# shunkenney/DPE-MVS

Measured on AMD Instinct MI355X. Metric: depth-map Mpixels/sec (9-view 1600x1200 PatchMatch) at 1/2/4/8 GPUs; L1 vs ref, higher is better.
Workload: dtype f32; 1 GPU; DTU-like 1600x1200, 9 src views, full-res REFINE_ITER pass + geometric consistency (BASELINE configs[2]); width=1600, height=1200, num_images=10, parallelism=reference-image sharding x1

## Files before the change

### dpe-mvs_amd/csrc/dpe_context.h

```cpp
#pragma once
#include <hip/hip_runtime.h>
#include <atomic>
#include <cstdint>
#include <map>
#include <memory>
#include <mutex>
#include <utility>
#include <vector>

#include "pass_common.h"
#include "tap_launch.h"
#include "dpe_fusion_types.h"
#include "cloud_dist.h"

namespace dpe {

inline std::atomic<long long> g_live_bytes{0};

template <class T>
struct DevArr {
  T* p = nullptr;
  size_t n = 0;
  DevArr() = default;
  DevArr(DevArr&& o) noexcept : p(o.p), n(o.n) { o.p = nullptr; o.n = 0; }
// ... 16 lines not shown
  void reset() {
    if (p) { g_live_bytes -= (long long)bytes(); (void)hipFree(p); }
    p = nullptr; n = 0;
  }
};

struct Stream {
  hipStream_t s = nullptr;
  Stream() = default;
  Stream(Stream&& o) noexcept : s(o.s) { o.s = nullptr; }
  Stream(const Stream&) = delete;
  Stream& operator=(const Stream&) = delete;
  ~Stream() { if (s) (void)hipStreamDestroy(s); }
  hipError_t create() { return hipStreamCreateWithFlags(&s, hipStreamNonBlocking); }
  operator hipStream_t() const { return s; }
};
struct Event {
  hipEvent_t e = nullptr;
  Event() = default;
  Event(Event&& o) noexcept : e(o.e) { o.e = nullptr; }
  Event(const Event&) = delete;
  Event& operator=(const Event&) = delete;
  ~Event() { if (e) (void)hipEventDestroy(e); }
  hipError_t create(unsigned flags = hipEventDisableTiming) { return hipEventCreateWithFlags(&e, flags); }
  operator hipEvent_t() const { return e; }
};

struct CachedImage {
  int id = 0, W = 0, H = 0;
  int cls = IMG_F32;
  DevArr<float> plain;
  DevArr<uint32_t> q8;
  DevArr<uint2> q16;
  DevArr<uint32_t> qp;
  DevArr<float4> qf;
  uint64_t last_use = 0;
  size_t bytes() const { return plain.n * 4 + q8.n * 4 + q16.n * 8 + qp.n * 4 + qf.n * 16; }
};

struct ResState {
  int w = 0, h = 0;
  bool full = false;
  DevArr<float4> planes;
  DevArr<uint8_t> weak;
  DevArr<uint32_t> sel;
  DevArr<float> snap;
  int snap_w = 0, snap_h = 0;
  bool has_snap = false;
};

struct PassWork {
  bool staged = false;
#if DPE_GN_ONCE
  bool gn_done_for_stage = false;
  DevArr<float> gn_complex;
#endif
  bool timing = false;
  bool counting = false;
  int gn_slots = 0;
  float timings[DPE_NUM_CLASSES + 1] = {0};
  int launches[DPE_NUM_CLASSES + 1] = {0};
  unsigned long long counts[DPE_NUM_CLASSES * 4] = {0};
  DevArr<unsigned long long> cnt;
  DevArr<unsigned long long> phase;
  PassConst hc;
  DevArr<PassConst> dc;
  DevArr<float> img_plain[DPE_MAX_IMAGES];
  DevArr<float4> imgq[DPE_MAX_IMAGES];
  DevArr<uint32_t> imgq8_all;
  DevArr<uint2> imgq16_all;
  DevArr<uint32_t> imgqp_all;
  int img_cls = IMG_F32;
  DevArr<float> depth[DPE_MAX_IMAGES];
  DevArr<uint8_t> edge, edge_low;
  DevArr<int> label;
  DevArr<float4> planes0;
  DevArr<uint8_t> weak0;
  DevArr<uint32_t> sel0;
  DevArr<float4> planes, planes_snap, fit_plane;
  DevArr<float> costs, costs_snap, complex_;
  DevArr<uint32_t> sel, sel_snap;
  DevArr<uint8_t> weak, weak_rel, vw;
  DevArr<short2> nb, nearest, edge_neigh, lab_bound;
  DevArr<int> radius;
  DevArr<int> tab_right, tab_down;
  DevArr<int> gn_ovf;
  DevArr<float> gn_tab;
  DevArr<int> lists, row_counts, list_totals;
  DevArr<int> part_cnt;
  DevBufs bufs;
};

struct EdgeScratch {
  DevArr<uint8_t> a, b, map;
  DevArr<float> fa, fb;
  DevArr<int> rows, mag, itab;
  DevArr<int16_t> dx, dy;
  DevArr<float> ftab;
  DevArr<short> stab;
};

struct FusionStage {
  std::vector<DevArr<float>> depth, normal;
  std::vector<FusionViewDev> host;
  DevArr<FusionViewDev> views;
  DevArr<DpeCamera> cams;
  DevArr<int> src;
  DevArr<int32_t> idx;
  DevArr<float> val;
  DevArr<uint8_t> cons_count;
  DevArr<float> cons_depth;
  int n = 0;
};

struct TatFusion {
  Event ev;
  std::vector<DevArr<uint8_t>> bgr, block, mask;
  DevArr<TatViewDev> views;
  bool ready = false;
  DevArr<float> dthr;
  DevArr<int> last, agg;
  DevArr<int> cnt, tot;
  DevArr<uint8_t> emit;
  DevArr<TatPoint> rec;
  DevArr<TatPoint> out[2];
  int turn = 0;
  bool copying = false;
  void views_restaged() { ready = false; }
};

struct VizScratch {
  std::mutex mu;
  std::map<const void*, Event> ev;
  DevArr<uint8_t> bgr;
  DevArr<int16_t> blocks;
  DevArr<uint16_t> q;
  int quality = 0;
  DevArr<float4> planes;
  DevArr<uint8_t> weak;
};

struct PointsScratch {
  std::mutex mu;
  std::map<const void*, Event> ev;
  DevArr<uint8_t> bgr;
  DevArr<int> cnt, tot;
  DevArr<TatPoint> out;
  DevArr<float4> planes;
  DevArr<uint8_t> weak;
};

struct CloudTimer {
  std::vector<Event> ev;
  std::vector<int> slot;
  bool on = false;
  float ms[4] = {0, 0, 0, 0};
  bool timed = false;
};
struct VoxelScratch {
  DevArr<uint8_t> rgb;
  DevArr<int4> cell;
  DevArr<uint32_t> frac;
  DevArr<int> owner, count;
  DevArr<uint32_t> first;
  DevArr<unsigned long long> sum, csum;
  DevArr<int> slot_at, bcnt;
// ... 78 lines not shown
```

### dpe-mvs_amd/csrc/dpe_mvs.hip

```cpp
#include <hip/hip_runtime.h>
#include <algorithm>
#include <cmath>
#include <cstdio>
#include <cstring>
#include <string>
#include <memory>
#include <utility>
#include <vector>

#include "pass_tables.h"
#include "pass_kernels.h"
#include "pass_refine.h"
#include "pass_sweep.h"
#include "tap_launch.h"
#include "dpe_entry.h"
#include "dpe_context.h"

using namespace dpe;

static const int kDefaultXcdRows = 1;
static constexpr int kWeakLanes = 16;

thread_local std::string dpe::g_err;

// ... 393 lines not shown
    } else {
      HIPC(c->pass.imgq[i].ensure(plane));
      TRY(build_f32_quads(c->stream, c->pass.img_plain[i].p, W, H, c->pass.imgq[i].p));
      B.imgq[i] = c->pass.imgq[i].p;
    }
  }
  B.ref = c->pass.img_plain[0].p;
  return DPE_OK;
}

static int stage_source_depths(DpeContext* c, const DpePassInput* in, const StageSrc& src) {
  const int W = in->width, H = in->height;
  const size_t L = (size_t)W * H;
  const dim3 rb2(32, 8), rg2((W + 31) / 32, (H + 7) / 8);
  for (int i = 1; i < in->num_images; ++i) {
    HIPC(c->pass.depth[i].ensure(L));
    if (src.st) {
      HIPC(hipMemcpyAsync(c->pass.depth[i].p, in->depths[i], L * sizeof(float), hipMemcpyHostToDevice, c->stream));
    } else {
      const ResState* r = src.dep[i];
      if (src.dep_snap)
        k_rescale_nearest<float><<<rg2, rb2, 0, c->stream>>>(r->snap.p, r->snap_w, r->snap_h, c->pass.depth[i].p, W, H, 0.0f);
      else
        k_rescale_depth<<<rg2, rb2, 0, c->stream>>>(r->planes.p, r->w, r->h, c->pass.depth[i].p, W, H);
      HIPC(hipGetLastError());
    }
    c->pass.bufs.depth[i] = c->pass.depth[i].p;
  }
  return DPE_OK;
}

static int stage_edge_label_maps(DpeContext* c, const DpePassInput* in) {
  const size_t L = (size_t)in->width * in->height, LL = (size_t)in->low_width * in->low_height;
  DevBufs& B = c->pass.bufs;
  if (in->params.use_edge || in->params.use_limit) {
    HIPC(c->pass.edge.ensure(L));
    HIPC(c->pass.edge_low.ensure(LL));
    HIPC(hipMemcpyAsync(c->pass.edge.p, in->edge, L, hipMemcpyHostToDevice, c->stream));
    HIPC(hipMemcpyAsync(c->pass.edge_low.p, in->edge_low_res, LL, hipMemcpyHostToDevice, c->stream));
    B.edge = c->pass.edge.p; B.edge_low = c->pass.edge_low.p;
  }
  if (in->params.use_label) {
    HIPC(c->pass.label.ensure(L));
    HIPC(hipMemcpyAsync(c->pass.label.p, in->label, L * sizeof(int), hipMemcpyHostToDevice, c->stream));
    B.label = c->pass.label.p;
  }
  return DPE_OK;
}

static int stage_initial_state(DpeContext* c, const DpePassInput* in, const StageSrc& src) {
  const DpePatchMatchParams& P = in->params;
  const int W = in->width, H = in->height;
  const size_t L = (size_t)W * H;
  HIPC(c->pass.planes0.ensure(L)); HIPC(c->pass.weak0.ensure(L)); HIPC(c->pass.sel0.ensure(L));
  if (const DpePassState* st = src.st) {
    HIPC(hipMemcpyAsync(c->pass.planes0.p, st->planes, L * sizeof(float4), hipMemcpyHostToDevice, c->stream));
    if (P.use_APD) HIPC(hipMemcpyAsync(c->pass.weak0.p, st->weak_info, L, hipMemcpyHostToDevice, c->stream));
    else HIPC(hipMemsetAsync(c->pass.weak0.p, DPE_STRONG, L, c->stream));
    HIPC(hipMemcpyAsync(c->pass.sel0.p, st->selected_views, L * sizeof(uint32_t), hipMemcpyHostToDevice, c->stream));
    return DPE_OK;
  }
  const ResState* r = src.prior;
  const dim3 rb2(32, 8), rg2((W + 31) / 32, (H + 7) / 8);
  if (P.state != DPE_FIRST_INIT) {
    k_rescale_nearest<float4><<<rg2, rb2, 0, c->stream>>>(r->planes.p, r->w, r->h, c->pass.planes0.p, W, H, make_float4(0, 0, 0, 0));
    k_rescale_nearest<uint32_t><<<rg2, rb2, 0, c->stream>>>(r->sel.p, r->w, r->h, c->pass.sel0.p, W, H, 0u);
  } else {
    HIPC(hipMemsetAsync(c->pass.planes0.p, 0, L * sizeof(float4), c->stream));
    HIPC(hipMemsetAsync(c->pass.sel0.p, 0, L * sizeof(uint32_t), c->stream));
  }
  if (P.use_APD) k_rescale_nearest<uint8_t><<<rg2, rb2, 0, c->stream>>>(r->weak.p, r->w, r->h, c->pass.weak0.p, W, H, (uint8_t)0);
  else HIPC(hipMemsetAsync(c->pass.weak0.p, DPE_STRONG, L, c->stream));
  HIPC(hipGetLastError());
  return DPE_OK;
}

static int ensure_working_set(DpeContext* c, int W, int H) {
  const size_t L = (size_t)W * H;
  HIPC(c->pass.planes.ensure(L)); HIPC(c->pass.planes_snap.ensure(L)); HIPC(c->pass.fit_plane.ensure(L));
  HIPC(c->pass.costs.ensure(L)); HIPC(c->pass.costs_snap.ensure(L)); HIPC(c->pass.complex_.ensure(L));
  HIPC(c->pass.sel.ensure(L)); HIPC(c->pass.sel_snap.ensure(L));
  HIPC(c->pass.weak.ensure(L)); HIPC(c->pass.weak_rel.ensure(L)); HIPC(c->pass.vw.ensure(L * DPE_MAX_IMAGES));
  HIPC(c->pass.nb.ensure(L * 9)); HIPC(c->pass.nearest.ensure(L)); HIPC(c->pass.edge_neigh.ensure(L * 8)); HIPC(c->pass.lab_bound.ensure(L * 8));
  HIPC(c->pass.radius.ensure(L));
  HIPC(c->pass.tab_right.ensure(L)); HIPC(c->pass.tab_down.ensure(L));
  HIPC(c->pass.gn_ovf.ensure(L + 64)); HIPC(c->pass.gn_tab.ensure((size_t)W + H));
  const PassLists lay(W, H, c->pass.hc.half_rows);
  HIPC(c->pass.lists.ensure((size_t)lay.lists_len())); HIPC(c->pass.row_counts.ensure(lay.row_counts_len()));
  HIPC(c->pass.list_totals.ensure(PassLists::kTotals)); HIPC(c->pass.part_cnt.ensure(lay.part_cnt_len()));
  DevBufs& B = c->pass.bufs;
  B.planes = c->pass.planes.p; B.planes_snap = c->pass.planes_snap.p; B.fit_plane = c->pass.fit_plane.p;
  B.planes0 = c->pass.planes0.p;
  B.costs = c->pass.costs.p; B.costs_snap = c->pass.costs_snap.p; B.complex_ = c->pass.complex_.p;
  B.sel = c->pass.sel.p; B.sel_snap = c->pass.sel_snap.p;
  B.weak = c->pass.weak.p; B.weak_rel = c->pass.weak_rel.p; B.vw = c->pass.vw.p;
  B.nb = c->pass.nb.p; B.nearest = c->pass.nearest.p; B.edge_neigh = c->pass.edge_neigh.p; B.lab_bound = c->pass.lab_bound.p;
  B.radius = c->pass.radius.p;
  return DPE_OK;
}

static int stage_impl(DpeContext* c, const DpePassInput* in, const StageSrc& src) {
  Range range_(src.st ? "dpe_pm_stage" : "dpe_pm_stage_resident");
  TRY(stage_check_args(in));
  HIPC(hipSetDevice(c->device));
  HIPC(wait_pending(c));
  set_pass_constants(c->pass.hc, in);
  HIPC(c->pass.dc.ensure(1));
  HIPC(hipMemcpyAsync(c->pass.dc.p, &c->pass.hc, sizeof(PassConst), hipMemcpyHostToDevice, c->stream));
  std::memset(&c->pass.bufs, 0, sizeof(c->pass.bufs));
  TRY(in->image_ids ? stage_images_cached(c, in) : stage_images_direct(c, in));
  if (in->params.geom_consistency) TRY(stage_source_depths(c, in, src));
  TRY(stage_edge_label_maps(c, in));
  TRY(stage_initial_state(c, in, src));
  TRY(ensure_working_set(c, in->width, in->height));
  HIPC(hipStreamSynchronize(c->stream));
  c->pass.staged = true;
#if DPE_GN_ONCE
  c->pass.gn_done_for_stage = false;
#endif
  return DPE_OK;
}

extern "C" int dpe_pm_stage(DpeContext* c, const DpePassInput* in, const DpePassState* st) {
  g_err.clear();
  if (!c || !in || !st || !in->images || !in->cams || !st->planes || !st->weak_info || !st->selected_views) {
    g_err = "dpe_pm_stage: null argument"; return DPE_ERR_ARG;
  }
  if (in->params.geom_consistency) {
    if (!in->depths) { g_err = "dpe_pm_stage: geom_consistency needs depths"; return DPE_ERR_ARG; }
    for (int i = 1; i < in->num_images; ++i) if (!in->depths[i]) { g_err = "dpe_pm_stage: missing source depth"; return DPE_ERR_ARG; }
  }
  StageSrc src;
  src.st = st;
  return stage_impl(c, in, src);
}

extern "C" int dpe_pm_stage_resident(DpeContext* c, const DpePassInput* in, int prior_id) {
  g_err.clear();
  if (!c || !in || !in->images || !in->cams) { g_err = "dpe_pm_stage_resident: null argument"; return DPE_ERR_ARG; }
  const DpePatchMatchParams& P = in->params;
  StageSrc src;
  auto find = [&](int id) -> const ResState* { auto it = c->rstore.find(id); return it == c->rstore.end() ? nullptr : &it->second; };
  if (P.state != DPE_FIRST_INIT || P.use_APD) {
    src.prior = find(prior_id);
    if (!src.prior || !src.prior->full) {
      g_err = "dpe_pm_stage_resident: no resident state of image " + std::to_string(prior_id); return DPE_ERR_STATE;
    }
  }
  if (P.geom_consistency) {
    if (!in->image_ids) { g_err = "dpe_pm_stage_resident: geom_consistency needs image_ids"; return DPE_ERR_ARG; }
    for (int i = 1; i < in->num_images && i < DPE_MAX_IMAGES; ++i) {
      src.dep[i] = find(in->image_ids[i]);
      if (!src.dep[i]) { g_err = "no depth map of source image " + std::to_string(in->image_ids[i]); return DPE_ERR_STATE; }
    }
    src.dep_snap = c->snap_mode;
    if (src.dep_snap)
      for (int i = 1; i < in->num_images && i < DPE_MAX_IMAGES; ++i)
        if (!src.dep[i]->has_snap) { g_err = "no depth snapshot of source image " + std::to_string(in->image_ids[i]); return DPE_ERR_STATE; }
  }
  return stage_impl(c, in, src);
}


static const char* const kClassName[DPE_NUM_CLASSES] = {"setup", "init", "strong", "ransac", "weak", "filter",
                                                         "depth_to_weak", "local_refine"};

struct PassRecorder {
  DpeContext* c = nullptr;
  hipStream_t s = nullptr;
  const DevBufs* base = nullptr;
  bool timing = false, slot_overflow = false;
  int max_slots = 0, nev = 0;
  std::vector<int> ev_class;

  int start(DpeContext* c_, hipStream_t s_, DevBufs& B) {
    c = c_; s = s_; base = &B;
    timing = c->pass.timing;
#if DPE_PHASE_PROF
    HIPC(c->pass.phase.ensure(32 * 64));
// ... 52 lines not shown
      }
    }
#if DPE_PHASE_PROF
    unsigned long long ph32[32 * 64], ph[64] = {};
    HIPC(hipMemcpyAsync(ph32, c->pass.phase.p, sizeof(ph32), hipMemcpyDeviceToHost, s));
    HIPC(hipStreamSynchronize(s));
    for (int k = 0; k < 32 * 64; ++k) ph[k % 64] += ph32[k];
    unsigned long long tot[4] = {0, 0, 0, 0};
    for (int k = 0; k < 64; ++k) tot[k / 16] += ph[k];
    for (int k = 0; k < 64; ++k)
      if (ph[k]) fprintf(stderr, "PHASE %d.%d %.4e cycles %.1f%%\n", k / 16, k % 16, (double)ph[k], 100.0 * ph[k] / tot[k / 16]);
#endif
    if (c->pass.counting) {
      HIPC(hipMemcpyAsync(c->pass.counts, c->pass.cnt.p, sizeof(c->pass.counts), hipMemcpyDeviceToHost, s));
      HIPC(hipStreamSynchronize(s));
      for (int k = 0; k < DPE_NUM_CLASSES; ++k) c->pass.counts[4 * k + 3] = (unsigned long long)c->pass.launches[k];
    }
    return DPE_OK;
  }
};
using Section = PassRecorder::Section;

struct PassRun {
  DpeContext* c;
  hipStream_t s, a;
  bool overlap;
  const PassConst& pc;
  const PassConst* dpc;
  DevBufs B;
  PassLists lay;
  size_t L;
  int nv;
  bool gn_skip = false;
  PassRecorder rec;

  PassRun(DpeContext* c_, hipStream_t s_)
      : c(c_), s(s_), a(s_), pc(c_->pass.hc), dpc(c_->pass.dc.p), B(c_->pass.bufs), lay(pc.W, pc.H, pc.half_rows),
        L((size_t)pc.W * pc.H), nv(pc.N - 1) {
    static const bool overlap_env = [] { const char* e = getenv("DPE_OVERLAP"); return !(e && atoi(e) == 0); }();
    overlap = overlap_env && !c->pass.timing && !c->pass.counting && pc.P.max_iterations >= 1;
    if (overlap) a = c->aux;
    B.cnt = nullptr;
    const char* e = getenv("DPE_XCD_ROWS");
    B.xcd_rows = e ? atoi(e) : kDefaultXcdRows;
  }
  hipError_t fork(hipEvent_t ev) const {
    const hipError_t e = overlap ? hipEventRecord(ev, s) : hipSuccess;
    return e != hipSuccess || !overlap ? e : hipStreamWaitEvent(a, ev, 0);
  }
  hipError_t aux_done(hipEvent_t ev) const { return overlap ? hipEventRecord(ev, a) : hipSuccess; }
  hipError_t wait_aux(hipEvent_t ev) const { return overlap ? hipStreamWaitEvent(s, ev, 0) : hipSuccess; }
  hipError_t join(hipEvent_t ev) const { const hipError_t e = aux_done(ev); return e != hipSuccess ? e : wait_aux(ev); }

  int* list(PassLists::Region r) const { return c->pass.lists.p + r.off; }
  int* rows(PassLists::Region r) const { return c->pass.row_counts.p + r.off; }
  int* total(int slot) const { return c->pass.list_totals.p + slot; }
  int* chunk_counts(int colour) const { return c->pass.part_cnt.p + lay.chunk_counts(colour).off; }
  dim3 px_grid() const { return dim3((pc.W + 15) / 16, (pc.H + 15) / 16); }
};
static const dim3 kPxBlock(16, 16);

template <int MODE>
static void build_lists(const PassRun& X, hipStream_t st, const DevBufs& Bl, PassLists::Region rows, int total,
                        PassLists::Region list) {
  const unsigned grid = (unsigned)(((MODE == 1 ? X.pc.H : X.pc.half_rows) + 3) / 4);
  const long stride = MODE == 1 ? X.lay.px() : list.len;
  int* rc = X.rows(rows);
  k_list_count<MODE><<<grid, 256, 0, st>>>(X.dpc, Bl, rc);
  k_list_scan<MODE><<<1, 64 * list_count<MODE>(), 0, st>>>(X.dpc, rc, X.total(total));
  k_list_fill<MODE><<<grid, 256, 0, st>>>(X.dpc, Bl, rc, X.list(list), stride);
}
static void sweep_lists(const PassRun& X, const DevBufs& Bl) {
  build_lists<0>(X, X.s, Bl, X.lay.sweep_rows(), PassLists::total_sweep(0, 0), X.lay.sweep(0, 0));
}

static int clear_setup_state(const PassRun& X, hipStream_t st) {
  const DevBufs& B = X.B;
  const size_t L = X.L;
  HIPC(hipMemsetAsync(B.fit_plane, 0, L * sizeof(float4), st));
  HIPC(hipMemsetAsync(B.complex_, 0, L * sizeof(float), st));
  if (!X.gn_skip) HIPC(hipMemsetAsync(B.weak_rel, 0xFF, L, st));
  if (!X.gn_skip) HIPC(hipMemsetAsync(B.nb, 0xFF, L * 9 * sizeof(short2), st));
  HIPC(hipMemsetAsync(B.nearest, 0xFF, L * sizeof(short2), st));
  HIPC(hipMemsetAsync(B.edge_neigh, 0xFF, L * 8 * sizeof(short2), st));
  HIPC(hipMemsetAsync(B.lab_bound, 0xFF, L * 8 * sizeof(short2), st));
  HIPC(hipMemsetAsync(B.radius, 0, L * sizeof(int), st));
  return DPE_OK;
}

static int gen_neighbours(PassRun& X, const DevBufs& Bc) {
  DpeContext* c = X.c;
  const hipStream_t a = X.a;
  const int* weak_list = X.list(X.lay.all_weak());
  const int* cnt = X.total(PassLists::kTotAllWeak);
  if (X.gn_skip) {
  } else if (X.pc.P.rotate_time <= 4) {
    int* ovf = X.total(PassLists::kTotGnOverflow);
    k_gn_tables<<<(unsigned)((X.pc.W + X.pc.H + 255) / 256), 256, 0, a>>>(X.dpc, c->pass.gn_tab.p);
    HIPC(hipMemsetAsync(ovf, 0, sizeof(int), a));
    const unsigned gg = (unsigned)((X.L + kGnBT - 1) / kGnBT);
    if (c->pass.gn_slots == 8)
      k_gen_neighbours_lds<8><<<gg, kGnBT, 0, a>>>(X.dpc, Bc, weak_list, cnt, c->pass.gn_tab.p, c->pass.gn_ovf.p, ovf);
    else if (X.pc.P.rotate_time <= 2 && c->pass.gn_slots != 64)
      k_gen_neighbours_lds<32><<<gg, kGnBT, 0, a>>>(X.dpc, Bc, weak_list, cnt, c->pass.gn_tab.p, c->pass.gn_ovf.p, ovf);
    else
      k_gen_neighbours_lds<64><<<gg, kGnBT, 0, a>>>(X.dpc, Bc, weak_list, cnt, c->pass.gn_tab.p, c->pass.gn_ovf.p, ovf);
    k_gen_neighbours<<<kGnOvfBlocks, 256, 0, a>>>(X.dpc, Bc, c->pass.gn_ovf.p, ovf);
  } else {
    k_gen_neighbours<<<kGnOvfBlocks, 256, 0, a>>>(X.dpc, Bc, weak_list, cnt);
  }
#if DPE_GN_ONCE
  if (!X.gn_skip) {
    HIPC(c->pass.gn_complex.ensure(X.L));
    HIPC(hipMemcpyAsync(c->pass.gn_complex.p, X.B.complex_, X.L * sizeof(float), hipMemcpyDeviceToDevice, a));
    c->pass.gn_done_for_stage = true;
  }
#endif
  return DPE_OK;
}

static int setup_chain(PassRun& X) {
  DpeContext* c = X.c;
  const PassConst& pc = X.pc;
  const hipStream_t a = X.a;
  Section sec(X.rec, DPE_CLASS_SETUP);
  const DevBufs& Bc = sec.B;
  if (X.overlap) sweep_lists(X, Bc);
  HIPC(X.fork(c->ev_fork));
  TRY(clear_setup_state(X, a));
  k_gen_edge_inform<<<X.px_grid(), kPxBlock, 0, a>>>(X.dpc, Bc);
  if (pc.P.use_edge) k_edge_rays<<<(unsigned)(3 * (pc.W + pc.H) - 2), 64, 0, a>>>(X.dpc, Bc);
#if DPE_GN_ONCE
  if (X.gn_skip) HIPC(hipMemcpyAsync(X.B.complex_, c->pass.gn_complex.p, X.L * sizeof(float), hipMemcpyDeviceToDevice, a));
#endif
  HIPC(X.aux_done(c->ev_ei));
  k_strong_tables_scan<<<(unsigned)(pc.W + pc.H), 64, 0, a>>>(X.dpc, Bc, c->pass.tab_right.p, c->pass.tab_down.p);
  k_find_nearest_strong<<<X.px_grid(), kPxBlock, 0, a>>>(X.dpc, Bc, c->pass.tab_right.p, c->pass.tab_down.p);
  build_lists<1>(X, a, Bc, X.lay.all_weak_rows(), PassLists::kTotAllWeak, X.lay.all_weak());
  TRY(gen_neighbours(X, Bc));
  k_neighbour_update<<<X.px_grid(), kPxBlock, 0, a>>>(X.dpc, Bc);
  if (X.overlap) build_lists<2>(X, a, Bc, X.lay.failed_rows(), PassLists::kTotFailed, X.lay.failed());
  else sweep_lists(X, Bc);
  HIPC(X.aux_done(c->ev_join));
  return DPE_OK;
}

static int random_initialization(PassRun& X) {
  {
    Section sec(X.rec, DPE_CLASS_INIT);
    if (X.c->pass.img_cls != IMG_F32) k_random_init<kTexInit><<<X.px_grid(), kPxBlock, 0, X.s>>>(X.dpc, sec.B);
    else k_random_init<TEX_F32><<<X.px_grid(), kPxBlock, 0, X.s>>>(X.dpc, sec.B);
  }
  HIPC(X.wait_aux(X.c->ev_ei));
  HIPC(hipGetLastError());
  return DPE_OK;
}

static void strong_sweep(const PassRun& X, const DevBufs& Bs, int it, PassLists::Region list, int total) {
  const bool edge = X.pc.P.use_edge;
  const int P = edge ? 4 : 8, C = edge ? 16 : 8;
  const size_t lds = (size_t)kBwStrong * strong_lds_per_wave(P, C, X.nv) * sizeof(float);
  const unsigned grid = (unsigned)((X.L / 2 + 1 + kBwStrong * P - 1) / (kBwStrong * P));
  launch_strong(edge, X.c->pass.img_cls, grid, lds, X.s, X.dpc, Bs, it, X.list(list), X.total(total));
}

static int strong_half_sweep(PassRun& X, int it, int colour) {
  const DevBufs& B = X.B;
// ... 174 lines not shown
```

### dpe-mvs_amd/csrc/pass_common.h

```cpp
#pragma once
#include "device_math.h"
#include "bres_walk.h"
#include "tex_addr.h"
#include "../../include/dpe_mvs.h"

namespace dpe {

struct ViewConst { float M[9]; float b[3]; };

struct PassConst {
  int W, H, N, LW, LH;
  int half_rows;
  uint32_t seed32, salt;
  float kinv0, kinv4, kc2, kc5;
  float gn_cos, gn_sin, gn_thr;
  int gn_shift;
  uint32_t gn_shift_m;
  int weak_nn;
  int tex_wide;
  float base_len[DPE_MAX_IMAGES];
  float spat36[36];
  DpePatchMatchParams P;
  DpeCamera cams[DPE_MAX_IMAGES];
  ViewConst vc[DPE_MAX_IMAGES];
};

struct DevBufs {
  const float4* imgq[DPE_MAX_IMAGES];
  const uint8_t* img8; uint32_t img8_view;
  const uint8_t* img16; uint32_t img16_view;
  const uint8_t* imgp; uint32_t imgp_view;
  const float* depth[DPE_MAX_IMAGES];
  const float* ref;
  float4* planes; float4* planes_snap; float4* fit_plane;
  const float4* planes0;
  float* costs; float* costs_snap; float* complex_;
  uint32_t* sel; uint32_t* sel_snap;
  uint8_t* weak; uint8_t* weak_rel; uint8_t* vw;
  short2* nb; short2* nearest; short2* edge_neigh; short2* lab_bound;
  int* radius;
  const uint8_t* edge; const uint8_t* edge_low; const int* label;
  unsigned long long* cnt;
  unsigned long long* phase;
  int xcd_rows;
};

#ifndef DPE_DIAG
#define DPE_DIAG 0
#endif
#define DPE_POOL_STATS (((DPE_DIAG) >> 4) & 1)
#define DPE_PHASE_PROF ((DPE_DIAG) & 1)
#define DPE_LINE_STATS (((DPE_DIAG) >> 1) & 1)
#define DPE_WEAK_STATS (((DPE_DIAG) >> 2) & 1)
#define DPE_GN_TIMES (((DPE_DIAG) >> 3) & 1)
#define DPE_FAKE_GATHER (((DPE_DIAG) >> 5) & 1)
#define DPE_GN_ONCE (((DPE_DIAG) >> 6) & 1)
#if DPE_PHASE_PROF
#define PHASE_BEGIN() uint64_t ph_t_ = __builtin_readcyclecounter(), ph_acc_[16] = {}
#define PHASE(k)                                                                    \
  do {                                                                              \
    const uint64_t n_ = __builtin_readcyclecounter();                               \
    ph_acc_[k] += n_ - ph_t_;                                                       \
    ph_t_ = n_;                                                                     \
  } while (0)
#define PHASE_END(kernel)                                                           \
  do {                                                                              \
    if ((threadIdx.x & 63) == 0 && B.phase)                                         \
      for (int k_ = 0; k_ < 16; ++k_)                                               \
        if (ph_acc_[k_]) atomicAdd(B.phase + ((blockIdx.x & 31) * 4 + (kernel)) * 16 + k_, (unsigned long long)ph_acc_[k_]); \
  } while (0)
#define PHASE_END_ALL(kernel)                                                       \
  do {                                                                              \
    if (B.phase)                                                                    \
      for (int k_ = 0; k_ < 16; ++k_)                                               \
        if (ph_acc_[k_]) atomicAdd(B.phase + ((blockIdx.x & 31) * 4 + (kernel)) * 16 + k_, (unsigned long long)ph_acc_[k_]); \
  } while (0)
#else
#define PHASE_BEGIN() do {} while (0)
#define PHASE(k) do {} while (0)
#define PHASE_END(kernel) do {} while (0)
#define PHASE_END_ALL(kernel) do {} while (0)
#endif
#if DPE_POOL_STATS
static __device__ unsigned long long g_pool[8][3];
DEV void pool_stat(int k, int jobs) {
  if ((threadIdx.x & 63) == 0) {
    atomicAdd(&g_pool[k][0], (unsigned long long)jobs);
    atomicAdd(&g_pool[k][1], (unsigned long long)((jobs + 63) / 64));
    atomicAdd(&g_pool[k][2], 1ull);
  }
}
#define POOL_STAT(k, n) pool_stat(k, n)
#define PATCH_STAT(ok) do { atomicAdd(&g_pool[6][0], 1ull); if (!(ok)) atomicAdd(&g_pool[6][1], 1ull); } while (0)
#else
#define POOL_STAT(k, n) do {} while (0)
#define PATCH_STAT(ok) do {} while (0)
#endif
DEV void count_work(const DevBufs& B, unsigned long long ncc, unsigned long long taps) {
  if (B.cnt) { atomicAdd(B.cnt + 0, ncc); atomicAdd(B.cnt + 1, taps); }
}

DEV int xcd_remap(int b, int nb, int chunk) {
  if (chunk <= 0) return b;
  const int super = 8 * chunk;
  const int S = (nb / super) * super;
  if (b >= S) return b;
  const int xcd = b & 7, pos = b >> 3;
  return ((pos / chunk) * 8 + xcd) * chunk + (pos % chunk);
}

DEV void setBit(uint32_t& v, unsigned n) { v |= (1u << n); }
DEV void unSetBit(uint32_t& v, unsigned n) { v &= (0xFFFFFFFEu << n); }
DEV int isSet(uint32_t v, unsigned n) { return (v >> n) & 1; }

DEV void normalize3(float4& v) {
  const float n2 = v.x * v.x + v.y * v.y + v.z * v.z;
  const float inv = d_rsqrtf(n2);
  v.x *= inv; v.y *= inv; v.z *= inv;
}
DEV void normalize2(float2& v) {
  const float n2 = v.x * v.x + v.y * v.y;
  const float inv = d_rsqrtf(n2);
// ... 749 lines not shown
```

### dpe-mvs_amd/csrc/pass_kernels.h

```cpp
#pragma once
#include "pass_common.h"

namespace dpe {

#define PIX2D_FULL()                                                   \
  const int lb_ = xcd_remap(blockIdx.y * gridDim.x + blockIdx.x, gridDim.x * gridDim.y, B.xcd_rows * gridDim.x); \
  const int x = (lb_ % gridDim.x) * blockDim.x + threadIdx.x;          \
  const int y = (lb_ / gridDim.x) * blockDim.y + threadIdx.y;          \
  if (x >= pc.W || y >= pc.H) return;                                  \
  const int center = x + y * pc.W;

#define PIX2D_HALF()                                                   \
  const int lb_ = xcd_remap(blockIdx.y * gridDim.x + blockIdx.x, gridDim.x * gridDim.y, B.xcd_rows * gridDim.x); \
  const int y = (lb_ / gridDim.x) * blockDim.y + threadIdx.y;          \
  const int x = 2 * ((lb_ % gridDim.x) * blockDim.x + threadIdx.x) + ((y + colour) & 1); \
  if (x >= pc.W || y >= pc.H || y >= pc.half_rows) return;             \
  const int center = x + y * pc.W;

constexpr int kEiTileR = 8, kEiTile = 16 + 2 * kEiTileR;
__global__ void __launch_bounds__(64) k_edge_rays(const PassConst* __restrict__ pcp, DevBufs B) {
  const PassConst& pc = *pcp;
  const int W = pc.W, H = pc.H;
  const int lane = threadIdx.x;
  int line = blockIdx.x;
  int f, x0, y0, sx, sy, len, iprev, inext;
  if (line < H) { f = 0; x0 = 0; y0 = line; sx = 1; sy = 0; len = W; iprev = 2; inext = 3; }
  else if ((line -= H) < W) { f = 1; x0 = line; y0 = 0; sx = 0; sy = 1; len = H; iprev = 0; inext = 1; }
  else if ((line -= W) < W + H - 1) {
    f = 2; const int c = line - (H - 1);
    y0 = c < 0 ? -c : 0; x0 = c + y0; sx = 1; sy = 1; len = MINo(H - y0, W - x0); iprev = 4; inext = 5;
  } else {
    line -= W + H - 1; f = 3; const int sm = line;
    y0 = sm - (W - 1) > 0 ? sm - (W - 1) : 0; x0 = sm - y0; sx = -1; sy = 1; len = MINo(H - y0, x0 + 1); iprev = 7; inext = 6;
  }
  (void)f;
  const unsigned long long below = lane == 0 ? 0ull : (~0ull >> (64 - lane));
  const unsigned long long above = lane == 63 ? 0ull : (~0ull << (lane + 1));
  int carry = -1;
  for (int t0 = 0; t0 < len; t0 += 64) {
    const int t = t0 + lane;
    const int px = x0 + t * sx, py = y0 + t * sy;
    const bool e = t < len && B.edge[py * W + px] != 0;
    const unsigned long long m = __ballot(e);
    const unsigned long long lo = m & below;
    const int prev = lo ? t0 + 63 - __builtin_clzll(lo) : carry;
    if (t < len) {
      B.edge_neigh[(size_t)(py * W + px) * 8 + iprev] =
          prev < 0 ? make_short2(-1, -1) : make_short2((short)(x0 + prev * sx), (short)(y0 + prev * sy));
    }
    if (m) carry = t0 + 63 - __builtin_clzll(m);
  }
  carry = -1;
  for (int t0 = ((len - 1) / 64) * 64; t0 >= 0; t0 -= 64) {
    const int t = t0 + lane;
    const int px = x0 + t * sx, py = y0 + t * sy;
    const bool e = t < len && B.edge[py * W + px] != 0;
    const unsigned long long m = __ballot(e);
    const unsigned long long hi = m & above;
    const int next = hi ? t0 + __builtin_ctzll(hi) : carry;
    if (t < len) {
      B.edge_neigh[(size_t)(py * W + px) * 8 + inext] =
          next < 0 ? make_short2(-1, -1) : make_short2((short)(x0 + next * sx), (short)(y0 + next * sy));
    }
    if (m) carry = t0 + __builtin_ctzll(m);
  }
}

__global__ void __launch_bounds__(256) k_gen_edge_inform(const PassConst* __restrict__ pcp, DevBufs B) {
  const PassConst& pc = *pcp;
  __shared__ uint8_t s_tile[kEiTile * kEiTile];
  __shared__ uint32_t s_hs[kEiTile][16];
  const int radius = pc.P.strong_radius;
  const bool tiled = pc.P.use_edge && radius >= 0 && radius <= kEiTileR && blockDim.x == 16;
  if (tiled) {
    const int lb0 = xcd_remap(blockIdx.y * gridDim.x + blockIdx.x, gridDim.x * gridDim.y, B.xcd_rows * gridDim.x);
    const int ox = (lb0 % gridDim.x) * blockDim.x - radius, oy = (lb0 / gridDim.x) * blockDim.y - radius;
    const int tw = blockDim.x + 2 * radius, th = blockDim.y + 2 * radius;
    for (int t = threadIdx.y * blockDim.x + threadIdx.x; t < tw * th; t += blockDim.x * blockDim.y) {
      const int nx = ox + t % tw, ny = oy + t / tw;
      uint8_t v = 0;
      if (nx >= 0 && nx < pc.W && ny >= 0 && ny < pc.H) {
        const int q = ny * pc.W + nx;
        v = 4 | (B.edge[q] ? 1 : 0) | ((pc.P.use_label && B.label[q] == 0) ? 2 : 0);
      }
      s_tile[t] = v;
    }
    __syncthreads();
    for (int t = threadIdx.y * blockDim.x + threadIdx.x; t < th * 16; t += blockDim.x * blockDim.y) {
      const uint8_t* row = s_tile + (t / 16) * tw + t % 16;
      uint32_t acc = 0;
      for (int i = 0; i <= 2 * radius; i++) {
        const uint32_t v = row[i];
        acc += (v & 1u) | ((v & 2u) << 9) | ((v & 4u) << 18);
      }
      s_hs[t / 16][t % 16] = acc;
    }
    __syncthreads();
  }
  PIX2D_FULL();
  const int W = pc.W, H = pc.H;
  if (pc.P.use_edge) {
    int edge_pix = 0, tot_pix = 0, bound_pix = 0;
    if (tiled) {
      uint32_t acc = 0;
      for (int j = 0; j <= 2 * radius; j++) acc += s_hs[threadIdx.y + j][threadIdx.x];
      edge_pix = (int)(acc & 1023u); bound_pix = (int)((acc >> 10) & 1023u); tot_pix = (int)(acc >> 20);
    } else {
      for (int i = -radius; i <= radius; i++)
        for (int j = -radius; j <= radius; j++) {
          const int nx = x + i, ny = y + j;
          if (nx < 0 || nx >= W || ny < 0 || ny >= H) continue;
          if (B.edge[ny * W + nx]) edge_pix++;
          if (pc.P.use_label && B.label[ny * W + nx] == 0) bound_pix++;
          tot_pix++;
        }
    }
    float density = 1.0f * edge_pix / tot_pix;
    if (pc.P.use_label) density = MAXo(density, (float)(bound_pix / tot_pix));
    B.complex_[center] = (float)(1.0f / (1.0f + d_exp_d(-25.0 * ((double)density - 0.35))));
  }
  if (pc.P.use_label && B.weak[center] == DPE_WEAK) {
    const int cl = B.label[center];
    if (cl > 0) {
      short2* lb = B.lab_bound + (size_t)center * 8;
      for (int i = 0; i < 8; i++) {
        const int dx = kDir[i][0], dy = kDir[i][1];
        const int sx = dx > 0 ? W - 1 - x : (dx < 0 ? x : 1 << 30);
        const int sy = dy > 0 ? H - 1 - y : (dy < 0 ? y : 1 << 30);
        const int n = MINo(sx, sy);
        int lk = -1;
        bool stop = false;
        for (int k0 = 1; k0 <= n && !stop; k0 += 8) {
          int lab[8];
#pragma unroll
          for (int k = 0; k < 8; ++k) lab[k] = (k0 + k <= n) ? B.label[(x + (k0 + k) * dx) + (y + (k0 + k) * dy) * W] : -1;
#pragma unroll
          for (int k = 0; k < 8; ++k) {
            if (stop) continue;
            if (k0 + k > n) { stop = true; continue; }
            if (lab[k] == cl) lk = k0 + k;
            else if (lab[k] == -1) stop = true;
          }
        }
        lb[i] = lk < 0 ? make_short2(-1, -1) : make_short2((short)(x + lk * dx), (short)(y + lk * dy));
      }
// ... 927 lines not shown
```

### dpe-mvs_amd/csrc/pass_sweep.h

```cpp
#pragma once
#include "pass_common.h"
#include "pass_refine.h"
#include "lds_layout.h"
#include "pass_lists.h"
#include "pool_tail.h"

namespace dpe {

template <int MODE> constexpr int list_count() { return MODE == 0 ? 4 : 1; }
template <int MODE> DEV int list_rows(const PassConst& pc) { return MODE == 1 ? pc.H : pc.half_rows; }
template <int MODE> DEV int list_key(const PassConst& pc, const DevBufs& B, int x, int y) {
  if constexpr (MODE == 2) return (((x + y) & 1) == 0 && B.weak_rel[y * pc.W + x] == 0) ? 0 : -1;
  const bool wk = B.weak[y * pc.W + x] == DPE_WEAK;
  if constexpr (MODE == 1) return wk ? 0 : -1;
  else return (((x + y) & 1) << 1) | (wk ? 1 : 0);
}
template <int MODE>
__global__ void k_list_count(const PassConst* __restrict__ pcp, DevBufs B, int* __restrict__ row_counts) {
  constexpr int NL = list_count<MODE>();
  const PassConst& pc = *pcp;
  const int wave = threadIdx.x >> 6, lane = threadIdx.x & 63;
  const int y = blockIdx.x * 4 + wave, rows = list_rows<MODE>(pc);
  if (y >= rows) return;
  int cnt[NL];
// ... 115 lines not shown
  int runA = 0;
  for (int i0 = base; i0 < min(n, base + kPartChunk); i0 += 256) {
    const int i = i0 + (int)threadIdx.x;
    const int p = i < n ? list[i] : 0;
    const int k = i < n ? part_key(pc, B, p) : 0;
    const unsigned long long m = __ballot(k == 1);
    if (lane == 0) s4[wave] = __popcll(m);
    __syncthreads();
    int a = runA + __popcll(m & below);
    for (int w = 0; w < wave; ++w) a += s4[w];
    const int all = s4[0] + s4[1] + s4[2] + s4[3];
    __syncthreads();
    if (i < n) out[k ? offA + a : offB + (i - base) - a] = p;
    runA += all;
  }
}

template <class CostF>
DEV float view_prob_raw(CostF cost, int i, float cost_threshold) {
  float count = 0; int count_false = 0; float tmpw = 0;
#pragma unroll
  for (int j = 0; j < 8; j++) {
    const float c = cost(j, i);
    if (c < cost_threshold) { tmpw += d_expf(c * c / (-0.18f)); count++; }
    if (c > 1.2f) count_false++;
  }
  float sp = 0.0f;
  if (count > 2 && count_false < 3) sp = tmpw / count;
  else if (count_false < 3) sp = d_expf(cost_threshold * cost_threshold / (-0.32f));
  return sp;
}

DEV void view_sample(const float* sp, int nv, Rng& rs, uint8_t* vw, uint32_t& tsv, float& wnorm) {
  for (int i = 0; i < DPE_MAX_IMAGES; ++i) vw[i] = 0;
  float psum = 0.0f;
  for (int i = 0; i < nv; ++i) psum += sp[i];
  const float inv = 1.0f / psum;
  float cdf[DPE_MAX_IMAGES];
  float cum = 0.0f;
  for (int i = 0; i < nv; ++i) { const float q = sp[i] * inv; cum += q; cdf[i] = cum; }
  for (int s = 0; s < 15; ++s) {
    const float rp = rng_uniform(rs) - 1.1920929e-07f;
    for (int id = 0; id < nv; ++id)
      if (cdf[id] > rp) { vw[id] += 1; break; }
  }
  uint32_t t = 0; float wn = 0;
  for (int i = 0; i < nv; ++i) if (vw[i] > 0) { setBit(t, i); wn += vw[i]; }
  tsv = t; wnorm = wn;
}

DEV void view_sample_coop(float* sp, int* cnt, int nv, int c, int C, bool active, const Rng& rs, uint8_t* vwl,
                          uint8_t* vwg) {
  if (active) {
    if (c == 0) {
      float psum = 0.0f;
      for (int i = 0; i < nv; ++i) psum += sp[i];
      const float inv = 1.0f / psum;
      float cum = 0.0f;
      for (int i = 0; i < nv; ++i) { const float q = sp[i] * inv; cum += q; sp[i] = cum; }
    }
    for (int v = c; v < nv; v += C) cnt[v] = 0;
  }
  wave_sync();
  if (active) {
    for (int s = c; s < 15; s += C) {
      const float rp = u32_to_uniform(rng_word(rs, (uint32_t)s)) - 1.1920929e-07f;
      for (int id = 0; id < nv; ++id)
        if (sp[id] > rp) { atomicAdd(&cnt[id], 1); break; }
    }
  }
  wave_sync();
  if (active)
    for (int j = c; j < DPE_MAX_IMAGES; j += C) {
      const uint8_t w = j < nv ? (uint8_t)cnt[j] : (uint8_t)0;
      vwl[j] = w;
      vwg[j] = w;
    }
  wave_sync();
}

DEV int edge_candidate(const PassConst& pc, const DevBufs& B, const float* __restrict__ costs, int x, int y, int center,
                       int iter, int d, int kind, bool on_edge) {
  const int W = pc.W, H = pc.H;
  const int dx = kDir[d][0], dy = kDir[d][1];
  const int s0 = MAXo(1, 5 - 2 * iter);
  const int min_step_len = 2;
  int step_num = 11, step_len = min_step_len;
  if (kind == 0) {
    const float max_edge_dist = MAXo(H, W) / 30.0f;
    const short2 ep = B.edge_neigh[(size_t)center * 8 + d];
    const double ex = (double)(ep.x - x), ey = (double)(ep.y - y);
    float dist = (float)__builtin_sqrt(ex * ex + ey * ey);
    if (d >= 4) dist = (float)((double)dist / 1.4142135623730951);
    if (on_edge) dist = 11 * min_step_len;
    else if (ep.x == -1 || ep.y == -1 || dist > max_edge_dist) {
      dist = max_edge_dist;
      if (d >= 4) dist = (float)((double)dist / 1.4142135623730951);
    }
    step_num = MINo(MAXo(11, f2i(1.0f * dist / min_step_len)), 22);
    step_len = MAXo(f2i(1.0f * dist / step_num), min_step_len);
    if (d < 4 && step_len % 2 == 1) step_len -= 1;
  }
  int fx = 0, fy = 0;
  if (d > 4) { if (d % 2) fx = dx; else fy = dy; }
  int mpos = -1; float mc = 3.40282347e+38f;
  for (int s = 0; s < step_num; s += 8) {
    float cv[8]; int pv[8]; bool ok[8];
#pragma unroll
    for (int u = 0; u < 8; ++u) {
      const int step = s + u;
      const int tx = x + s0 * dx + step * step_len * dx + fx, ty = y + s0 * dy + step * step_len * dy + fy;
      ok[u] = step < step_num && tx >= 0 && ty >= 0 && tx < W && ty < H;
      pv[u] = tx + ty * W;
      cv[u] = ok[u] ? costs[pv[u]] : 0.0f;
    }
#pragma unroll
    for (int u = 0; u < 8; ++u)
      if (ok[u] && mc > cv[u]) { mpos = pv[u]; mc = cv[u]; }
  }
  return mc < 3.40282347e+38f ? mpos : -1;
}

DEV int acmh_candidate(const PassConst& pc, const float* __restrict__ costs, int x, int y, int center, int s) {
  const int W = pc.W, H = pc.H;
  float costMin; int cmp;
  switch (s) {
    case 1: {
      if (!(y > 2)) return -1;
      const int up_far = center - 3 * W; costMin = costs[up_far]; cmp = up_far;
      for (int i = 1; i < 11; ++i) if (y > 2 + 2 * i) { const int pt = up_far - 2 * i * W; if (costs[pt] < costMin) { costMin = costs[pt]; cmp = pt; } }
      return cmp;
    }
    case 3: {
      if (!(y < H - 3)) return -1;
      const int down_far = center + 3 * W; costMin = costs[down_far]; cmp = down_far;
      for (int i = 1; i < 11; ++i) if (y < H - 3 - 2 * i) { const int pt = down_far + 2 * i * W; if (costs[pt] < costMin) { costMin = costs[pt]; cmp = pt; } }
      return cmp;
    }
    case 5: {
      if (!(x > 2)) return -1;
      const int left_far = center - 3; costMin = costs[left_far]; cmp = left_far;
      for (int i = 1; i < 11; ++i) if (x > 2 + 2 * i) { const int pt = left_far - 2 * i; if (costs[pt] < costMin) { costMin = costs[pt]; cmp = pt; } }
      return cmp;
    }
    case 7: {
      if (!(x < W - 3)) return -1;
      const int right_far = center + 3; costMin = costs[right_far]; cmp = right_far;
      for (int i = 1; i < 11; ++i) if (x < W - 3 - 2 * i) { const int pt = right_far + 2 * i; if (costs[pt] < costMin) { costMin = costs[pt]; cmp = pt; } }
      return cmp;
    }
    case 0: {
      if (!(y > 0)) return -1;
      const int up_near = center - W; costMin = costs[up_near]; cmp = up_near;
      for (int i = 0; i < 3; ++i) {
        if (y > 1 + i && x > i) { const int pt = up_near - (1 + i) * W - (1 + i); if (costs[pt] < costMin) { costMin = costs[pt]; cmp = pt; } }
        if (y > 1 + i && x < W - 1 - i) { const int pt = up_near - (1 + i) * W + (1 + i); if (costs[pt] < costMin) { costMin = costs[pt]; cmp = pt; } }
      }
      return cmp;
    }
    case 2: {
      if (!(y < H - 1)) return -1;
      const int down_near = center + W; costMin = costs[down_near]; cmp = down_near;
      for (int i = 0; i < 3; ++i) {
        if (y < H - 2 - i && x > i) { const int pt = down_near + (1 + i) * W - (1 + i); if (costs[pt] < costMin) { costMin = costs[pt]; cmp = pt; } }
        if (y < H - 2 - i && x < W - 1 - i) { const int pt = down_near + (1 + i) * W + (1 + i); if (costs[pt] < costMin) { costMin = costs[pt]; cmp = pt; } }
      }
      return cmp;
    }
    case 4: {
      if (!(x > 0)) return -1;
      const int left_near = center - 1; costMin = costs[left_near]; cmp = left_near;
      for (int i = 0; i < 3; ++i) {
        if (x > 1 + i && y > i) { const int pt = left_near - (1 + i) - (1 + i) * W; if (costs[pt] < costMin) { costMin = costs[pt]; cmp = pt; } }
        if (x > 1 + i && y < H - 1 - i) { const int pt = left_near - (1 + i) + (1 + i) * W; if (costs[pt] < costMin) { costMin = costs[pt]; cmp = pt; } }
      }
      return cmp;
    }
    default: {
      if (!(x < W - 1)) return -1;
      const int right_near = center + 1; costMin = costs[right_near]; cmp = right_near;
      for (int i = 0; i < 3; ++i) {
        if (x < W - 2 - i && y > i) { const int pt = right_near + (1 + i) - (1 + i) * W; if (costs[pt] < costMin) { costMin = costs[pt]; cmp = pt; } }
        if (x < W - 2 - i && y < H - 1 - i) { const int pt = right_near + (1 + i) + (1 + i) * W; if (costs[pt] < costMin) { costMin = costs[pt]; cmp = pt; } }
      }
      return cmp;
    }
  }
}

constexpr int kTailJobs = kTailLdsJobs;
template <int P, int C> using StrongCarveT = lds::StrongCarve<P, C, kTailJobs>;
__host__ __device__ inline int strong_lds_per_wave(int P, int C, int nv) {
  return P == 4 && C == 16 ? StrongCarveT<4, 16>::total(nv) : StrongCarveT<8, 8>::total(nv);
}
template <int P, int C>
struct StrongWave {
  using SC = StrongCarveT<P, C>;
  float* wl;
  int nv;
  DEV float4* hyp(int q) const { return (float4*)(wl + SC::hyp()) + q * 5; }
  DEV float* patch(int q) const { return wl + SC::patch() + q * SC::kPatch; }
  DEV float* cost(int q) const { return wl + SC::cost(nv) + q * (C + 1) * nv; }
  DEV float* sp(int q) const { return wl + SC::sp(nv) + q * nv; }
// ... 1110 lines not shown
```

Baseline: 31.72 Mpix/s.

## Precompute edge-scan step geometry in scan kernel and use prefix bounds in candidate search

The edge-scan kernel now derives each pixel's step count and step length from the distance to the nearest edge along each direction. It uses a shared-memory lookup table indexed by distance and stores the result as a packed 16-bit value per pixel and direction. edge_candidate reads this packed value instead of loading edge_neigh and computing sqrt and divisions per candidate. It also computes the in-bounds step prefix once, so the per-step bounds checks go away and the last valid load is clamped. The memset of edge_neigh is dropped, and the scan kernel writes an extra buffer.

```diff
diff --git a/dpe-mvs_amd/csrc/dpe_context.h b/dpe-mvs_amd/csrc/dpe_context.h
--- a/dpe-mvs_amd/csrc/dpe_context.h
+++ b/dpe-mvs_amd/csrc/dpe_context.h
@@ -122,6 +122,7 @@
   DevArr<uint32_t> sel, sel_snap;
   DevArr<uint8_t> weak, weak_rel, vw;
   DevArr<short2> nb, nearest, edge_neigh, lab_bound;
+  DevArr<uint16_t> scan_geo;
   DevArr<int> radius;
   DevArr<int> tab_right, tab_down;
   DevArr<int> gn_ovf;
diff --git a/dpe-mvs_amd/csrc/dpe_mvs.hip b/dpe-mvs_amd/csrc/dpe_mvs.hip
--- a/dpe-mvs_amd/csrc/dpe_mvs.hip
+++ b/dpe-mvs_amd/csrc/dpe_mvs.hip
@@ -499,6 +499,7 @@
   HIPC(c->pass.sel.ensure(L)); HIPC(c->pass.sel_snap.ensure(L));
   HIPC(c->pass.weak.ensure(L)); HIPC(c->pass.weak_rel.ensure(L)); HIPC(c->pass.vw.ensure(L * DPE_MAX_IMAGES));
   HIPC(c->pass.nb.ensure(L * 9)); HIPC(c->pass.nearest.ensure(L)); HIPC(c->pass.edge_neigh.ensure(L * 8)); HIPC(c->pass.lab_bound.ensure(L * 8));
+  HIPC(c->pass.scan_geo.ensure(L * 8));
   HIPC(c->pass.radius.ensure(L));
   HIPC(c->pass.tab_right.ensure(L)); HIPC(c->pass.tab_down.ensure(L));
   HIPC(c->pass.gn_ovf.ensure(L + 64)); HIPC(c->pass.gn_tab.ensure((size_t)W + H));
@@ -512,6 +513,7 @@
   B.sel = c->pass.sel.p; B.sel_snap = c->pass.sel_snap.p;
   B.weak = c->pass.weak.p; B.weak_rel = c->pass.weak_rel.p; B.vw = c->pass.vw.p;
   B.nb = c->pass.nb.p; B.nearest = c->pass.nearest.p; B.edge_neigh = c->pass.edge_neigh.p; B.lab_bound = c->pass.lab_bound.p;
+  B.scan_geo = c->pass.scan_geo.p;
   B.radius = c->pass.radius.p;
   return DPE_OK;
 }
@@ -730,7 +732,6 @@
   if (!X.gn_skip) HIPC(hipMemsetAsync(B.weak_rel, 0xFF, L, st));
   if (!X.gn_skip) HIPC(hipMemsetAsync(B.nb, 0xFF, L * 9 * sizeof(short2), st));
   HIPC(hipMemsetAsync(B.nearest, 0xFF, L * sizeof(short2), st));
-  HIPC(hipMemsetAsync(B.edge_neigh, 0xFF, L * 8 * sizeof(short2), st));
   HIPC(hipMemsetAsync(B.lab_bound, 0xFF, L * 8 * sizeof(short2), st));
   HIPC(hipMemsetAsync(B.radius, 0, L * sizeof(int), st));
   return DPE_OK;
diff --git a/dpe-mvs_amd/csrc/pass_common.h b/dpe-mvs_amd/csrc/pass_common.h
--- a/dpe-mvs_amd/csrc/pass_common.h
+++ b/dpe-mvs_amd/csrc/pass_common.h
@@ -2,6 +2,7 @@
 #include "device_math.h"
 #include "bres_walk.h"
 #include "tex_addr.h"
+#include "scan_geo.h"
 #include "../../include/dpe_mvs.h"
 
 namespace dpe {
@@ -38,6 +39,7 @@
   uint32_t* sel; uint32_t* sel_snap;
   uint8_t* weak; uint8_t* weak_rel; uint8_t* vw;
   short2* nb; short2* nearest; short2* edge_neigh; short2* lab_bound;
+  uint16_t* scan_geo;
   int* radius;
   const uint8_t* edge; const uint8_t* edge_low; const int* label;
   unsigned long long* cnt;
diff --git a/dpe-mvs_amd/csrc/pass_kernels.h b/dpe-mvs_amd/csrc/pass_kernels.h
--- a/dpe-mvs_amd/csrc/pass_kernels.h
+++ b/dpe-mvs_amd/csrc/pass_kernels.h
@@ -33,7 +33,16 @@
     line -= W + H - 1; f = 3; const int sm = line;
     y0 = sm - (W - 1) > 0 ? sm - (W - 1) : 0; x0 = sm - y0; sx = -1; sy = 1; len = MINo(H - y0, x0 + 1); iprev = 7; inext = 6;
   }
-  (void)f;
+  __shared__ uint16_t s_geo[kScanLutMax];
+  const int dcls = f >= 2 ? 4 : 0;
+  const int nfar = scan_geo_far_len(W, H), nlut = MINo(nfar, kScanLutMax);
+  for (int n = lane; n < nlut; n += 64) s_geo[n] = scan_geo_pack(edge_scan_geometry(W, H, 0, 0, n, f >= 2 ? n : 0, dcls));
+  const uint16_t geo_far = scan_geo_pack(edge_scan_geometry(W, H, 0, 0, -1, -1, dcls));
+  __syncthreads();
+  auto geo_at = [&](int n) -> uint16_t {
+    if (n < 0 || n >= nfar) return geo_far;
+    return n < nlut ? s_geo[n] : scan_geo_pack(edge_scan_geometry(W, H, 0, 0, n, f >= 2 ? n : 0, dcls));
+  };
   const unsigned long long below = lane == 0 ? 0ull : (~0ull >> (64 - lane));
   const unsigned long long above = lane == 63 ? 0ull : (~0ull << (lane + 1));
   int carry = -1;
@@ -45,8 +54,9 @@
     const unsigned long long lo = m & below;
     const int prev = lo ? t0 + 63 - __builtin_clzll(lo) : carry;
     if (t < len) {
-      B.edge_neigh[(size_t)(py * W + px) * 8 + iprev] =
-          prev < 0 ? make_short2(-1, -1) : make_short2((short)(x0 + prev * sx), (short)(y0 + prev * sy));
+      const short2 ep = prev < 0 ? make_short2(-1, -1) : make_short2((short)(x0 + prev * sx), (short)(y0 + prev * sy));
+      B.edge_neigh[(size_t)(py * W + px) * 8 + iprev] = ep;
+      B.scan_geo[(size_t)(py * W + px) * 8 + iprev] = geo_at(prev < 0 ? -1 : t - prev);
     }
     if (m) carry = t0 + 63 - __builtin_clzll(m);
   }
@@ -59,8 +69,9 @@
     const unsigned long long hi = m & above;
     const int next = hi ? t0 + __builtin_ctzll(hi) : carry;
     if (t < len) {
-      B.edge_neigh[(size_t)(py * W + px) * 8 + inext] =
-          next < 0 ? make_short2(-1, -1) : make_short2((short)(x0 + next * sx), (short)(y0 + next * sy));
+      const short2 ep = next < 0 ? make_short2(-1, -1) : make_short2((short)(x0 + next * sx), (short)(y0 + next * sy));
+      B.edge_neigh[(size_t)(py * W + px) * 8 + inext] = ep;
+      B.scan_geo[(size_t)(py * W + px) * 8 + inext] = geo_at(next < 0 ? -1 : next - t);
     }
     if (m) carry = t0 + __builtin_ctzll(m);
   }
diff --git a/dpe-mvs_amd/csrc/pass_sweep.h b/dpe-mvs_amd/csrc/pass_sweep.h
--- a/dpe-mvs_amd/csrc/pass_sweep.h
+++ b/dpe-mvs_amd/csrc/pass_sweep.h
@@ -221,43 +221,30 @@
 DEV int edge_candidate(const PassConst& pc, const DevBufs& B, const float* __restrict__ costs, int x, int y, int center,
                        int iter, int d, int kind, bool on_edge) {
   const int W = pc.W, H = pc.H;
-  const int dx = kDir[d][0], dy = kDir[d][1];
   const int s0 = MAXo(1, 5 - 2 * iter);
-  const int min_step_len = 2;
-  int step_num = 11, step_len = min_step_len;
-  if (kind == 0) {
-    const float max_edge_dist = MAXo(H, W) / 30.0f;
-    const short2 ep = B.edge_neigh[(size_t)center * 8 + d];
-    const double ex = (double)(ep.x - x), ey = (double)(ep.y - y);
-    float dist = (float)__builtin_sqrt(ex * ex + ey * ey);
-    if (d >= 4) dist = (float)((double)dist / 1.4142135623730951);
-    if (on_edge) dist = 11 * min_step_len;
-    else if (ep.x == -1 || ep.y == -1 || dist > max_edge_dist) {
-      dist = max_edge_dist;
-      if (d >= 4) dist = (float)((double)dist / 1.4142135623730951);
-    }
-    step_num = MINo(MAXo(11, f2i(1.0f * dist / min_step_len)), 22);
-    step_len = MAXo(f2i(1.0f * dist / step_num), min_step_len);
-    if (d < 4 && step_len % 2 == 1) step_len -= 1;
-  }
-  int fx = 0, fy = 0;
-  if (d > 4) { if (d % 2) fx = dx; else fy = dy; }
-  int mpos = -1; float mc = 3.40282347e+38f;
-  for (int s = 0; s < step_num; s += 8) {
-    float cv[8]; int pv[8]; bool ok[8];
+  ScanGeo g{kScanFixedNum, kScanFixedLen};
+  if (kind == 0 && !on_edge) g = scan_geo_unpack(B.scan_geo[(size_t)center * 8 + d]);
+  int dx, dy;
+  scan_dir(d, dx, dy);
+  const int kmax = scan_prefix(x, y, d, s0, g.step_len, g.step_num, W, H);
+  const int dpos = dx + dy * W;
+  int p0 = center + s0 * dpos;
+  if (d > 4) p0 += (d & 1) ? dx : dy * W;
+  const int stride = g.step_len * dpos;
+  const int p0b = p0 * 4, strideb = stride * 4;
+  uint32_t moff = 0; float mc = 3.40282347e+38f;
+  for (int s = 0; s < kmax; s += 8) {
+    float cv[8]; uint32_t off[8];
 #pragma unroll
     for (int u = 0; u < 8; ++u) {
-      const int step = s + u;
-      const int tx = x + s0 * dx + step * step_len * dx + fx, ty = y + s0 * dy + step * step_len * dy + fy;
-      ok[u] = step < step_num && tx >= 0 && ty >= 0 && tx < W && ty < H;
-      pv[u] = tx + ty * W;
-      cv[u] = ok[u] ? costs[pv[u]] : 0.0f;
+      off[u] = (uint32_t)(p0b + __mul24(MINo(s + u, kmax - 1), strideb));
+      cv[u] = *(const float*)((const char*)costs + off[u]);
     }
 #pragma unroll
     for (int u = 0; u < 8; ++u)
-      if (ok[u] && mc > cv[u]) { mpos = pv[u]; mc = cv[u]; }
-  }
-  return mc < 3.40282347e+38f ? mpos : -1;
+      if (mc > cv[u]) { moff = off[u]; mc = cv[u]; }
+  }
+  return mc < 3.40282347e+38f ? (int)(moff >> 2) : -1;
 }
 
 DEV int acmh_candidate(const PassConst& pc, const float* __restrict__ costs, int x, int y, int center, int s) {
diff --git a/dpe-mvs_amd/csrc/scan_geo.h b/dpe-mvs_amd/csrc/scan_geo.h
--- /dev/null
+++ b/dpe-mvs_amd/csrc/scan_geo.h
@@ -0,0 +1,73 @@
+#pragma once
+#include <cstdint>
+
+#if defined(__HIPCC__)
+#define SCAN_HD __host__ __device__ __forceinline__
+#else
+#define SCAN_HD inline
+#endif
+
+namespace dpe {
+
+constexpr int kScanMinStepLen = 2;
+constexpr int kScanFixedNum = 11, kScanFixedLen = kScanMinStepLen;
+struct ScanGeo { int step_num, step_len; };
+
+SCAN_HD uint16_t scan_geo_pack(ScanGeo g) { return (uint16_t)(g.step_num | g.step_len << 8); }
+SCAN_HD ScanGeo scan_geo_unpack(uint16_t v) { return ScanGeo{v & 0xFF, v >> 8}; }
+
+SCAN_HD void scan_dir(int d, int& dx, int& dy) {
+  dx = (int)((0x8885u >> (2 * d)) & 3u) - 1;
+  dy = (int)((0x2858u >> (2 * d)) & 3u) - 1;
+}
+
+SCAN_HD int scan_f2i(float f) {
+  if (f != f) return 0;
+  if (f >= 2147483520.0f) return 2147483647;
+  if (f <= -2147483648.0f) return (int)0x80000000;
+  return (int)f;
+}
+
+SCAN_HD ScanGeo edge_scan_geometry(int W, int H, int x, int y, int epx, int epy, int d) {
+  const float max_edge_dist = (H < W ? W : H) / 30.0f;
+  const double ex = (double)(epx - x), ey = (double)(epy - y);
+  float dist = (float)__builtin_sqrt(ex * ex + ey * ey);
+  if (d >= 4) dist = (float)((double)dist / 1.4142135623730951);
+  if (epx == -1 || epy == -1 || dist > max_edge_dist) {
+    dist = max_edge_dist;
+    if (d >= 4) dist = (float)((double)dist / 1.4142135623730951);
+  }
+  const int n = scan_f2i(1.0f * dist / kScanMinStepLen);
+  ScanGeo g;
+  g.step_num = n < 11 ? 11 : (n > 22 ? 22 : n);
+  const int l = scan_f2i(1.0f * dist / g.step_num);
+  g.step_len = l < kScanMinStepLen ? kScanMinStepLen : l;
+  if (d < 4 && g.step_len % 2 == 1) g.step_len -= 1;
+  return g;
+}
+
+SCAN_HD int scan_geo_far_len(int W, int H) { return scan_f2i((H < W ? W : H) / 30.0f) + 2; }
+constexpr int kScanLutMax = 544;
+
+SCAN_HD int scan_prefix(int x, int y, int d, int s0, int step_len, int step_num, int W, int H) {
+  int dx, dy;
+  scan_dir(d, dx, dy);
+  const int ax = s0 + ((d > 4 && (d & 1)) ? 1 : 0), ay = s0 + ((d > 4 && !(d & 1)) ? 1 : 0);
+  const int cap = step_num * step_len;
+  const int rx = dx > 0 ? W - 1 - x - ax : (dx < 0 ? x - ax : cap);
+  const int ry = dy > 0 ? H - 1 - y - ay : (dy < 0 ? y - ay : cap);
+  int r = rx < ry ? rx : ry;
+  if (r < 0) return 0;
+  if (r > cap) r = cap;
+#if defined(__HIP_DEVICE_COMPILE__)
+  int q = (int)((float)r * __builtin_amdgcn_rcpf((float)step_len));
+#else
+  int q = (int)((float)r * (1.0f / (float)step_len));
+#endif
+  const int rem = r - q * step_len;
+  if (rem < 0) q -= 1;
+  else if (rem >= step_len) q += 1;
+  return q + 1 < step_num ? q + 1 : step_num;
+}
+
+}
```

New measurement: 31.89 Mpix/s, median of 6. About the same (+0.5%).
